# ericzzj1989/BALF

Hardware: NVIDIA B200
Metric: images/sec detect+NMS+top-k @640x480 (higher is better)
Workload: dtype fp16/tf32 operands (11-bit significand), fp32 accumulate

## Files before the change

### balf_b200/csrc/detector_tc.cuh

```cuda
#pragma once
#include <cuda_fp16.h>
#include "detector.cuh"
#include "umma.cuh"

namespace balf {
using namespace umma;

constexpr int kMerge32Ctas = 3;
constexpr int kRc16MinC = 32;
constexpr int TM = 128;
constexpr int NT2 = 256;
constexpr int kMaxSlot = 4;
constexpr int kMaxGemm = 6;

struct TcGemm {
    uint32_t goff;
    uint16_t nblk;
    uint16_t rows;
    uint16_t kb;
    uint16_t bias;
    uint16_t h16;
};
__host__ __device__ constexpr uint32_t tc_eb(int h16) { return h16 == 1 ? 2u : 4u; }
struct TcPlan {
// ... 107 lines not shown
    static constexpr int nslot = PX ? (C == 256 ? 2 : 3) : (C == 256 ? 3 : 2);
    __host__ __device__ static constexpr int rows(int gi) { return gi == BG_WM ? 64 : C; }
    __host__ __device__ static constexpr int K(int gi) { return gi == BG_CONV0 ? tc_kin(CIN) : gi == BG_WM ? 64 : C; }
    __host__ __device__ static constexpr bool bias(int gi) { return gi != BG_WM; }
    __host__ __device__ static constexpr bool h16(int gi) { return gi != BG_CONV0 || CIN >= 8; }
};
template <int CIN, int C, int PX = 0> struct MergeG {
    static constexpr int count = MG_COUNT;
    static constexpr bool x3 = PX != 0;
    static constexpr bool ebias = C == 128 && PX == 0;
    static constexpr bool resident = PX ? C <= 32 : C <= 128;
    static constexpr int cap = 32768;
    static constexpr int nslot = PX ? (C == 64 ? 3 : 2) : (C == 256 ? 2 : 3);
    __host__ __device__ static constexpr int rows(int) { return C; }
    __host__ __device__ static constexpr int K(int gi) { return gi == MG_CONV0 ? tc_kin(CIN) : C; }
    __host__ __device__ static constexpr bool bias(int gi) { return !ebias && gi != MG_PD2A; }
    __host__ __device__ static constexpr bool h16(int gi) {
        return gi == MG_PD2A || gi == MG_PD2B || (gi == MG_CONV0 && CIN >= 8) || ((gi == MG_RC1 || gi == MG_RC2) && (PX || C > kRc16MinC));
    }
};
template <int C, int PX = 0> struct HeadG {
    static constexpr int count = HG_COUNT;
    static constexpr bool x3 = PX != 0;
    static constexpr bool resident = false;
    static constexpr int cap = 32768;
    static constexpr int nslot = 2;
    __host__ __device__ static constexpr int rows(int gi) { return gi == HG_DENSE ? kHeadN : C; }
    __host__ __device__ static constexpr int K(int) { return C; }
    __host__ __device__ static constexpr bool bias(int) { return true; }
    __host__ __device__ static constexpr bool h16(int) { return true; }
};
template <typename G> __host__ __device__ constexpr int g_mode(int gi) { return G::h16(gi) ? (G::x3 ? 2 : 1) : 0; }
template <typename G> __host__ __device__ constexpr uint32_t g_bytes(int gi) {
    return (uint32_t)G::rows(gi) * (G::K(gi) * tc_eb(g_mode<G>(gi)) + (G::bias(gi) ? 32u : 0u));
}
template <typename G> __host__ __device__ constexpr uint32_t g_off(int gi) { uint32_t o = 0; for (int i = 0; i < gi; ++i) o += g_bytes<G>(i); return o; }

constexpr uint32_t kDescHi = (128u >> 4) | (1u << 14);
__device__ __forceinline__ uint64_t desc_of(uint32_t addr, uint32_t lbo) {
    return ((uint64_t)kDescHi << 32) | (uint64_t)(((lbo >> 4) << 16) | ((addr >> 4) & 0x3FFFu));
}

__host__ __device__ constexpr uint32_t make_idesc_f16(int M, int N) { return (1u << 4) | ((uint32_t)(N >> 3) << 17) | ((uint32_t)(M >> 4) << 24); }
__device__ __forceinline__ void mma_f16(uint32_t d_tmem, uint64_t a_desc, uint64_t b_desc, uint32_t idesc, bool accumulate) {
    asm volatile(
        "{\n\t.reg .pred p;\n\tsetp.ne.b32 p, %4, 0;\n\t"
        "tcgen05.mma.cta_group::1.kind::f16 [%0], %1, %2, %3, p;\n\t}"
        :: "r"(d_tmem), "l"(a_desc), "l"(b_desc), "r"(idesc), "r"((uint32_t)accumulate) : "memory");
}
constexpr uint32_t kDescHiSw = (1024u >> 4) | (1u << 14) | (2u << 29);
__device__ __forceinline__ uint64_t desc_sw_of(uint32_t addr) {
    return ((uint64_t)kDescHiSw << 32) | (uint64_t)((1u << 16) | ((addr >> 4) & 0x3FFFu));
}
template <typename G, int GI, bool ASW = false>
__device__ __forceinline__ void issue_linear_t(Ring& r, const TcPlan& p, uint32_t a_addr, uint32_t ones_addr, uint32_t d_tmem, bool first) {
    constexpr int ROWS = G::rows(GI), K = G::K(GI);
    constexpr bool BIAS = G::bias(GI), H16 = G::h16(GI);
    constexpr bool X3 = H16 && G::x3;
    static_assert(!(H16 && ASW), "fp16 operands use the chunk-major layout");
    constexpr int KB = tc_kb(ROWS, K, G::cap, (int)tc_eb(g_mode<G>(GI))), NBLK = K / KB;
    constexpr uint32_t idesc = H16 ? make_idesc_f16(128, ROWS) : make_idesc_tf32(128, ROWS);
    constexpr uint32_t a_lbo = TM * 16u, b_lbo = (uint32_t)ROWS * 16u;
    constexpr int KSTEP = H16 ? 16 : 8, EPC = H16 ? 8 : 4;
    const uint64_t a_desc = ASW ? desc_sw_of(a_addr) : desc_of(a_addr, a_lbo);
#pragma unroll
    for (int b = 0; b < NBLK; ++b) {
        uint32_t w_addr, slot = 0;
        if (G::resident) {
            w_addr = r.wsm + g_off<G>(GI) + (uint32_t)b * ROWS * KB * tc_eb(g_mode<G>(GI));
        } else {
            ring_top_up<G::nslot>(r, p);
            slot = r.cslot;
            mbar_wait(&r.full[slot], r.cpar);
            w_addr = r.wsm + slot * p.slot_bytes;
        }
        const uint64_t b_desc = desc_of(w_addr, b_lbo);
        fence_after_sync();
#pragma unroll
        for (int ks = 0; ks < KB / KSTEP; ++ks) {
            const uint32_t kchunk = (uint32_t)(b * KB) / EPC + (uint32_t)ks * 2u;
            const uint32_t a_off = ASW ? (kchunk / 8u) * (TM * 128u) + (kchunk % 8u) * 16u : kchunk * a_lbo;
            if (H16) mma_f16(d_tmem, a_desc + (a_off >> 4), b_desc + (((uint32_t)ks * 2u * b_lbo) >> 4), idesc, !(first && b == 0 && ks == 0));
            else mma_tf32(d_tmem, a_desc + (a_off >> 4), b_desc + (((uint32_t)ks * 2u * b_lbo) >> 4), idesc, !(first && b == 0 && ks == 0));
            if constexpr (X3) {
                mma_f16(d_tmem, a_desc + ((a_off + (uint32_t)(K / 8) * a_lbo) >> 4), b_desc + (((uint32_t)ks * 2u * b_lbo) >> 4), idesc, true);
                mma_f16(d_tmem, a_desc + (a_off >> 4), b_desc + ((((uint32_t)KB / 8u + (uint32_t)ks * 2u) * b_lbo) >> 4), idesc, true);
            }
        }
        if (BIAS && b + 1 == NBLK)
            mma_tf32(d_tmem, desc_of(ones_addr, TM * 16u), b_desc + ((((uint32_t)KB / EPC) * (X3 ? 2u : 1u) * b_lbo) >> 4), make_idesc_tf32(128, ROWS), true);
        if (!G::resident) { commit(&r.empty[slot]); ring_consumed<G::nslot>(r); }
    }
}

constexpr uint32_t kDescHiMn = ((uint32_t)(TM * 16u) >> 4) | (1u << 14);
__device__ __forceinline__ uint64_t desc_mn_of(uint32_t addr) {
    return ((uint64_t)kDescHiMn << 32) | (uint64_t)(((128u >> 4) << 16) | ((addr >> 4) & 0x3FFFu));
}
template <typename G, int GI, int C>
__device__ __forceinline__ void issue_mix_t(Ring& r, const TcPlan& p, uint32_t y_addr, uint32_t d_tmem) {
    uint32_t w_addr, slot = 0;
    if (G::resident) {
        w_addr = r.wsm + g_off<G>(GI);
    } else {
        ring_top_up<G::nslot>(r, p);
        slot = r.cslot;
        mbar_wait(&r.full[slot], r.cpar);
        w_addr = r.wsm + slot * p.slot_bytes;
    }
    fence_after_sync();
    constexpr uint32_t idesc = make_idesc_f16(64, C) | (1u << 16);
    constexpr uint32_t lo_off = (uint32_t)(C / 8) * TM * 16u;
    const uint64_t w_desc = desc_of(w_addr, 1024u);
    const uint64_t y_desc = desc_mn_of(y_addr);
#pragma unroll
    for (uint32_t u = 0; u < 2; ++u) {
#pragma unroll
        for (uint32_t ks = 0; ks < 4; ++ks) {
            const uint32_t yo = (32u * ks + 16u * u) * 16u;
            mma_f16(d_tmem + ((u * 16u) << 16), w_desc + ((ks * 2u * 1024u) >> 4), y_desc + (yo >> 4), idesc, ks > 0);
            if constexpr (G::x3) {
                mma_f16(d_tmem + ((u * 16u) << 16), w_desc + ((ks * 2u * 1024u) >> 4), y_desc + ((lo_off + yo) >> 4), idesc, true);
                mma_f16(d_tmem + ((u * 16u) << 16), w_desc + ((8192u + ks * 2u * 1024u) >> 4), y_desc + (yo >> 4), idesc, true);
            }
        }
    }
    if (!G::resident) { commit(&r.empty[slot]); ring_consumed<G::nslot>(r); }
}

__device__ __forceinline__ float ex2_approx(float x) {
    float y;
    asm("ex2.approx.ftz.f32 %0, %1;" : "=f"(y) : "f"(x));
    return y;
}
// ... 62 lines not shown
template <int CH>
__device__ __forceinline__ void st_row(uint32_t taddr, const float (&v)[CH]) {
    if constexpr (CH == 16) {
        asm volatile(
            "tcgen05.st.sync.aligned.32x32b.x16.b32 [%0], {%1, %2, %3, %4, %5, %6, %7, %8, %9, %10, %11, %12, %13, %14, %15, %16};"
            :: "r"(taddr), "r"(__float_as_uint(v[0])), "r"(__float_as_uint(v[1])), "r"(__float_as_uint(v[2])), "r"(__float_as_uint(v[3])),
               "r"(__float_as_uint(v[4])), "r"(__float_as_uint(v[5])), "r"(__float_as_uint(v[6])), "r"(__float_as_uint(v[7])),
               "r"(__float_as_uint(v[8])), "r"(__float_as_uint(v[9])), "r"(__float_as_uint(v[10])), "r"(__float_as_uint(v[11])),
               "r"(__float_as_uint(v[12])), "r"(__float_as_uint(v[13])), "r"(__float_as_uint(v[14])), "r"(__float_as_uint(v[15]))
            : "memory");
    } else {
#pragma unroll
        for (int c0 = 0; c0 < CH; c0 += 32) tmem_st32(taddr + c0, *reinterpret_cast<const float (*)[32]>(&v[c0]));
    }
    tmem_st_wait();
}

template <int CH>
__device__ __forceinline__ void row_to_a(const float (&v)[CH], float* region, int row, int col0) {
#pragma unroll
    for (int j = 0; j < CH / 4; ++j)
        *reinterpret_cast<float4*>(region + ((size_t)(col0 / 4 + j) * TM + row) * 4) =
            to_tf32(make_float4(v[4 * j], v[4 * j + 1], v[4 * j + 2], v[4 * j + 3]));
}

__device__ __forceinline__ void split_h2(float a, float b, uint32_t& hi, uint32_t& lo) {
    asm("cvt.rn.satfinite.f16x2.f32 %0, %1, %2;" : "=r"(hi) : "f"(b), "f"(a));
    const float2 f = __half22float2(*reinterpret_cast<const __half2*>(&hi));
    asm("cvt.rn.satfinite.f16x2.f32 %0, %1, %2;" : "=r"(lo) : "f"(b - f.y), "f"(a - f.x));
}
template <int CH, int LOC = 0>
__device__ __forceinline__ void row_to_a16(const float (&v)[CH], float* region, int row, int col0) {
#pragma unroll
    for (int j = 0; j < CH / 8; ++j) {
        uint32_t h[4], l[4];
#pragma unroll
        for (int e = 0; e < 4; ++e) {
            if constexpr (LOC > 0) split_h2(v[8 * j + 2 * e], v[8 * j + 2 * e + 1], h[e], l[e]);
            else asm("cvt.rn.satfinite.f16x2.f32 %0, %1, %2;" : "=r"(h[e]) : "f"(v[8 * j + 2 * e + 1]), "f"(v[8 * j + 2 * e]));
        }
        *reinterpret_cast<uint4*>(region + ((size_t)(col0 / 8 + j) * TM + row) * 4) = make_uint4(h[0], h[1], h[2], h[3]);
        if constexpr (LOC > 0) *reinterpret_cast<uint4*>(region + ((size_t)(LOC + col0 / 8 + j) * TM + row) * 4) = make_uint4(l[0], l[1], l[2], l[3]);
    }
}

__host__ __device__ __forceinline__ int sw_off(int row, int chunk) { return (chunk >> 3) * (TM * 32) + row * 32 + (((chunk & 7) ^ (row & 7)) << 2); }
template <int CH, bool ROUND>
__device__ __forceinline__ void row_to_sw(const float (&v)[CH], float* region, int row, int col0) {
#pragma unroll
    for (int j = 0; j < CH / 4; ++j) {
        float4 o = make_float4(v[4 * j], v[4 * j + 1], v[4 * j + 2], v[4 * j + 3]);
        if (ROUND) o = to_tf32(o);
        *reinterpret_cast<float4*>(region + sw_off(row, col0 / 4 + j)) = o;
    }
}
__device__ __forceinline__ void bulk_store(const float* gdst, uint32_t ssrc, uint32_t bytes) {
    asm volatile("cp.async.bulk.global.shared::cta.bulk_group [%0], [%1], %2;" :: "l"(gdst), "r"(ssrc), "r"(bytes) : "memory");
}
__device__ __forceinline__ void bulk_commit() { asm volatile("cp.async.bulk.commit_group;" ::: "memory"); }
__device__ __forceinline__ void bulk_wait_read() { asm volatile("cp.async.bulk.wait_group.read 0;" ::: "memory"); }
__device__ __forceinline__ void bulk_wait_all() { asm volatile("cp.async.bulk.wait_group 0;" ::: "memory"); }

template <int NG, int NTG = NT2>
__device__ __forceinline__ void group_sync(int grp) {
    if constexpr (NG == 1) __syncthreads();
    else asm volatile("bar.sync %0, %1;" :: "r"(grp + 1), "n"(NTG) : "memory");
}

template <int NG = 1, int TPR = 2>
__device__ __forceinline__ void row_stats(float sum, float sq, float2* xch, int row, int half, int C, float& rstd, float& shift, int grp = 0) {
    if constexpr (TPR == 2) {
        xch[half * TM + row] = make_float2(sum, sq);
        group_sync<NG, TM * TPR>(grp);
        const float2 o = xch[(half ^ 1) * TM + row];
        sum += o.x; sq += o.y;
    } else if constexpr (TPR > 2) {
        xch[half * TM + row] = make_float2(sum, sq);
        group_sync<NG, TM * TPR>(grp);
        sum = 0.f; sq = 0.f;
#pragma unroll
        for (int p = 0; p < TPR; ++p) { const float2 o = xch[p * TM + row]; sum += o.x; sq += o.y; }
    }
    const float inv_c = C == 32 ? 1.0f / 32 : C == 64 ? 1.0f / 64 : C == 128 ? 1.0f / 128 : 1.0f / 256;
    const float mean = sum * inv_c;
    const float var = fmaxf(sq * inv_c - mean * mean, 0.f);
    rstd = rsqrtf(var + 1e-5f);
    shift = -mean * rstd;
}

struct TcShared {
    float* region;
    uint32_t wsm;
    float* ones;
    float2* xch;
    float* vec;
    uint2* sched;
    uint64_t* full;
    uint64_t* empty;
    uint64_t* done;
    uint64_t* aux;
    uint32_t* tmem_slot;
    uint64_t* gdone;
};
constexpr int kMaxGroups = 8;
constexpr uint32_t kSchedEntries = 62;
constexpr uint32_t kOnesBytes = 2 * TM * 16, kXchBytes = 2 * 2 * TM * 8, kVecBytes = (2 * 256 + 64) * 4, kSchedBytes = (kSchedEntries + 2) * 8, kTcTail = 256;
// ... 308 lines not shown
#pragma unroll
                for (int q = 0; q < 4; ++q) {
                    if constexpr (H16 == 2) split_h2(e[2 * q], e[2 * q + 1], h[q], l[q]);
                    else asm("cvt.rn.satfinite.f16x2.f32 %0, %1, %2;" : "=r"(h[q]) : "f"(e[2 * q + 1]), "f"(e[2 * q]));
                }
                *reinterpret_cast<uint4*>(dst + ((size_t)((half * N + j) / 2) * TM + row) * 4) = make_uint4(h[0], h[1], h[2], h[3]);
                if constexpr (H16 == 2)
                    *reinterpret_cast<uint4*>(dst + ((size_t)(CIN / 8 + (half * N + j) / 2) * TM + row) * 4) = make_uint4(l[0], l[1], l[2], l[3]);
            } else {
                *reinterpret_cast<float4*>(dst + ((size_t)(half * N + j) * TM + row) * 4) = to_tf32(c0);
                *reinterpret_cast<float4*>(dst + ((size_t)(half * N + j + 1) * TM + row) * 4) = to_tf32(c1);
            }
        }
    }
}


constexpr int kConv0Off = 64;
template <int CIN, int C>
__device__ __forceinline__ void conv0_stage_weights(const DownW& w, float* vec) {
    for (int i = threadIdx.x; i < CIN * C; i += NT2) vec[kConv0Off + i] = __ldg(w.conv0_w + i);
    for (int i = threadIdx.x; i < C; i += NT2) vec[kConv0Off + CIN * C + i] = __ldg(w.conv0_b + i);
}
template <int CIN, int C, int CH>
__device__ __forceinline__ void conv0_row(const float4 x, const float* vec, int col0, float (&v)[CH]) {
    const float xs[4] = {x.x, x.y, x.z, x.w};
    const float* cw = vec + kConv0Off + col0;
#pragma unroll
    for (int i = 0; i < CH; i += 4) {
        const float4 b = *reinterpret_cast<const float4*>(cw + CIN * C + i);
        unsigned long long a01 = pk2(b.x, b.y), a23 = pk2(b.z, b.w);
#pragma unroll
        for (int k = 0; k < CIN; ++k) {
            const float4 wv = *reinterpret_cast<const float4*>(cw + k * C + i);
            const unsigned long long xk = pk2(xs[k], xs[k]);
            a01 = fma2(pk2(wv.x, wv.y), xk, a01);
            a23 = fma2(pk2(wv.z, wv.w), xk, a23);
        }
        upk2(a01, v[i], v[i + 1]);
        upk2(a23, v[i + 2], v[i + 3]);
#pragma unroll
        for (int j = 0; j < 4; ++j) v[i + j] = fmaxf(v[i + j], 0.f);
    }
}

template <int C, int PX> struct BranchCfg {
    static constexpr int TPR = C == 32 ? 1 : C == 256 ? 4 : 2;
    static constexpr int groups = C == 32 ? 5 : C == 64 ? 2 : 1;
    static constexpr int NTG = TM * TPR;
    static constexpr int CH = C / TPR;
    static constexpr uint32_t region = (uint32_t)TM * C * (PX ? 4u : 2u);
    static constexpr bool park_u = C <= 128;
    static constexpr bool h16_out = C <= 128;
    static constexpr int col_u = 0;
    static constexpr int col_y = park_u ? C : 0;
    static constexpr int ncols = groups * tc_cols(col_y + 2 * C) > 512 ? col_y + 2 * C : tc_cols(col_y + 2 * C);
    static constexpr uint32_t xch = TPR == 1 ? 0u : 2u * TPR * TM * 8u;
    static constexpr int SC = TPR == 1 ? 16 : TPR == 4 ? (CH < 32 ? CH : 32) : (CH > 64 ? 64 : CH);
};

template <int CIN, int C, int BR, int PX>
__device__ __forceinline__ void tc_branch_body(const float* __restrict__ xin, const DownW& w, const TcPlan& plan, const UnitGeom& geo,
                                               float* __restrict__ out, float* __restrict__ scratch, unsigned char* smem) {
    using Cfg = BranchCfg<C, PX>;
    using G = BranchG<CIN, C, PX>;
    constexpr int CH = Cfg::CH, NG = Cfg::groups, TPR = Cfg::TPR, NTG = Cfg::NTG, SC = Cfg::SC;
    constexpr bool X3 = PX != 0;
    constexpr int LOC = X3 ? C / 8 : 0;
    constexpr bool XH = !X3 && CIN >= 8;
    constexpr bool CL16 = !Cfg::h16_out && !X3;
    float* const rt = CL16 ? scratch : out;
    constexpr int XM = XH ? 3 : X3 ? 2 : 1;
    static_assert(NG == 1 || G::resident, "tile groups share resident weights (no ring state per group)");
    static_assert(CH % SC == 0 && SC % 16 == 0, "sub-chunking");
    TcShared s = carve(smem, Cfg::region, plan, NG, Cfg::xch);
    const int grp = NG == 1 ? 0 : (int)(threadIdx.x / NTG);
    const int tid = threadIdx.x - grp * NTG, row = tid & (TM - 1), half = tid >> 7;
    const int vblock = (int)blockIdx.x * NG + grp, vgrid = (int)gridDim.x * NG;
    const int ntiles = (geo.total_units + 1) / 2;
    const uint32_t my_tiles = vblock < ntiles ? (ntiles - 1 - vblock) / vgrid + 1 : 0;
    const DownW::Branch& br = w.br[BR];
    if (grp == 0) {
        for (int i = tid; i < C; i += NTG) { s.vec[i] = __ldg(br.gn_w + i); s.vec[256 + i] = __ldg(br.gn_b + i); }
        for (int i = tid; i < 64; i += NTG) s.vec[512 + i] = __ldg(br.gd_b + i) + 1.0f;
        if constexpr (CIN < 8) {
            for (int i = tid; i < CIN * C; i += NTG) s.vec[kConv0Off + i] = __ldg(w.conv0_w + i);
            for (int i = tid; i < C; i += NTG) s.vec[kConv0Off + CIN * C + i] = __ldg(w.conv0_b + i);
        }
    }
    Ring ring;
    const bool w0 = __shfl_sync(0xffffffffu, tid >> 5, 0) == 0;
    tc_prologue<G::nslot>(s, tc_cols(Cfg::ncols * NG), ring, plan, my_tiles, w0 && grp == 0);
    if (NG > 1) {
        if (grp > 0 && w0 && elect_one()) mbar_wait(&s.full[0], 0);
        s.region += (size_t)grp * (Cfg::region / 4);
        s.xch += (size_t)grp * (Cfg::xch / 8);
        if (grp > 0) s.done = &s.gdone[grp];
    }
    const uint32_t tm = *s.tmem_slot + (uint32_t)(grp * Cfg::ncols);
    const uint32_t lane_base = tm + ((uint32_t)(row & ~31) << 16);
    const uint32_t region_addr = smem_u32(s.region), ones_addr = smem_u32(s.ones);
    const int ug = (row & 31) >> 4, tok = (row >> 5) * 16 + (row & 15);
    const int col0 = half * CH;
    const float* const mix_b1p = s.vec + 512 + tok;
    const int ostride = (BR == 0 ? geo.fw : 1) * C;
    const size_t npix = (size_t)geo.h * geo.w;
    uint32_t phase = 0, xb = 0;
    int it = 0;
    InputPf<CIN, TPR> pf;
    auto coords = [&](int tt, bool& vld, int& im, int& px) {
        const int un = 2 * tt + ug;
        vld = un < geo.total_units;
        im = vld ? fast_div(un, geo.upi, geo.inv_upi) : 0;
        px = unit_pixel<BR>(geo, vld ? un - im * geo.upi : 0, tok);
    };
    auto stats_of = [&](const float (&v)[CH], float& sum, float& sq) {
        unsigned long long s2 = pk2(0.f, 0.f), q2 = pk2(0.f, 0.f);
#pragma unroll
        for (int i = 0; i < CH; i += 2) {
            const unsigned long long x = pk2(v[i], v[i + 1]);
            s2 = add2(s2, x); q2 = fma2(x, x, q2);
        }
        float a, b;
        upk2(s2, a, b); sum = a + b;
        upk2(q2, a, b); sq = a + b;
    };
    bool nvld = false; int nim = 0, npx = 0;
// ... 67 lines not shown
            commit(s.done);
        }
        TC_TRACE(plan, it, 8);
        wait_done_ring<G, NG, NTG>(s.done, phase, ring, plan, w0, grp);
        TC_TRACE(plan, it, 9);
        {
            ld_row<CH>(lane_base + Cfg::col_y + col0, v);
            { float d0, d1; gelu_row<CH, false>(v, d0, d1); }
            st_row<CH>(lane_base + Cfg::col_y + col0, v);
            ld_row<CH>(lane_base + Cfg::col_y + C + col0, v);
            float sum = 0.f, sq = 0.f;
            gelu_row<CH, true>(v, sum, sq);
            row_stats<NG, TPR>(sum, sq, s.xch + (xb++ & 1) * TPR * TM, row, half, C, rstd, shift, grp);
            norm_row<CH>(v, rstd, shift);
#pragma unroll
            for (int i = 0; i < CH; i += 4) {
                const float4 gw = *reinterpret_cast<const float4*>(s.vec + col0 + i), gb = *reinterpret_cast<const float4*>(s.vec + 256 + col0 + i);
                upk2(fma2(pk2(v[i], v[i + 1]), pk2(gw.x, gw.y), pk2(gb.x, gb.y)), v[i], v[i + 1]);
                upk2(fma2(pk2(v[i + 2], v[i + 3]), pk2(gw.z, gw.w), pk2(gb.z, gb.w)), v[i + 2], v[i + 3]);
            }
            row_to_a16<CH, LOC>(v, s.region, row, col0);
        }
        TC_TRACE(plan, it, 10);
        sync_for_mma<NG, NTG>(grp);
        if (w0 && elect_one()) { issue_mix_t<G, BG_WM, C>(ring, plan, region_addr, tm + Cfg::col_y + C); commit(s.done); }
        TC_TRACE(plan, it, 11);
        wait_done_ring<G, NG, NTG>(s.done, phase, ring, plan, w0, grp);
        TC_TRACE(plan, it, 12);
        {
#pragma unroll 1
            for (int c = 0; c < CH; c += SC) {
                float y1[SC], y2[SC];
                ld_row<SC>(lane_base + Cfg::col_y + col0 + c, y1);
                ld_row<SC>(lane_base + Cfg::col_y + C + col0 + c, y2);
                const float mix_b1 = *mix_b1p;
                const unsigned long long b2 = pk2(mix_b1, mix_b1);
#pragma unroll
                for (int i = 0; i < SC; i += 2) upk2(mul2(pk2(y1[i], y1[i + 1]), add2(pk2(y2[i], y2[i + 1]), b2)), y2[i], y2[i + 1]);
                row_to_a16<SC, LOC>(y2, s.region, row, col0 + c);
            }
        }
        TC_TRACE(plan, it, 13);
        sync_for_mma<NG, NTG>(grp);
        if (w0 && elect_one()) { issue_linear_t<G, BG_D2>(ring, plan, region_addr, ones_addr, tm + Cfg::col_y, true); commit(s.done); }
        TC_TRACE(plan, it, 14);
        wait_done_ring<G, NG, NTG>(s.done, phase, ring, plan, w0, grp);
        TC_TRACE(plan, it, 15);
        {
            const bool odd = (threadIdx.x & 1) != 0;
            const size_t own_base = Cfg::h16_out ? ((size_t)img * npix + (pix & ~(TM - 1))) * C * (X3 ? 2 : 1)
                                                 : ((size_t)img * npix + pix) * C;
            const size_t oth_base = __shfl_xor_sync(0xffffffffu, (unsigned long long)own_base, 1);
            const size_t base_a = odd ? oth_base : own_base, base_b = odd ? own_base : oth_base;
            if constexpr (CL16 && CH % 64 == 0) {
                float hv[CH / 2];
#pragma unroll
                for (int c = 0; c < CH; c += SC) {
                    float a[SC];
                    ld_row<SC>(lane_base + Cfg::col_y + col0 + c, a);
#pragma unroll
                    for (int j0 = 0; j0 < SC / 4; j0 += 8) {
                        float4 t8[8];
                        pair_load<8>(reinterpret_cast<const float4*>(orow + c) + j0, valid, t8);
#pragma unroll
                        for (int j = 0; j < 8; j += 2) {
                            pair_unswap(t8[j], t8[j + 1]);
#pragma unroll
                            for (int u2 = 0; u2 < 2; ++u2) {
                                const float4 rr = t8[j + u2];
                                const int i = 4 * (j0 + j + u2);
                                uint32_t h0, h1;
                                asm("cvt.rn.satfinite.f16x2.f32 %0, %1, %2;" : "=r"(h0) : "f"(a[i + 1] + rr.y), "f"(a[i] + rr.x));
                                asm("cvt.rn.satfinite.f16x2.f32 %0, %1, %2;" : "=r"(h1) : "f"(a[i + 3] + rr.w), "f"(a[i + 2] + rr.z));
                                hv[(c + i) / 2] = __uint_as_float(h0);
                                hv[(c + i) / 2 + 1] = __uint_as_float(h1);
                            }
                        }
                    }
                }
                oct_store<CH / 8>(out, (((size_t)img * npix + pix) * C + col0) / 2, ostride / 2, hv, valid);
            } else
#pragma unroll 1
            for (int c = 0; c < CH; c += SC) {
                float a[SC], r[SC];
                ld_row<SC>(lane_base + Cfg::col_y + col0 + c, a);
                if (Cfg::park_u) ld_row<SC>(lane_base + Cfg::col_u + col0 + c, r);
                if constexpr (Cfg::h16_out) {
                    __half* tile = reinterpret_cast<__half*>(out) + own_base + (size_t)(pix & (TM - 1)) * 8;
#pragma unroll
                    for (int j = 0; j < SC / 8; ++j) {
                        uint32_t h[4], l[4];
#pragma unroll
                        for (int e = 0; e < 4; ++e) {
                            float lo, hi;
                            upk2(add2(pk2(a[8 * j + 2 * e], a[8 * j + 2 * e + 1]), pk2(r[8 * j + 2 * e], r[8 * j + 2 * e + 1])), lo, hi);
                            if constexpr (X3) split_h2(lo, hi, h[e], l[e]);
                            else asm("cvt.rn.satfinite.f16x2.f32 %0, %1, %2;" : "=r"(h[e]) : "f"(hi), "f"(lo));
                        }
                        if (valid) {
                            *reinterpret_cast<uint4*>(tile + (size_t)((col0 + c) / 8 + j) * (TM * 8)) = make_uint4(h[0], h[1], h[2], h[3]);
                            if constexpr (X3)
                                *reinterpret_cast<uint4*>(tile + (size_t)(C / 8 + (col0 + c) / 8 + j) * (TM * 8)) = make_uint4(l[0], l[1], l[2], l[3]);
                        }
                    }
                    continue;
                }
                float4 o[SC / 4];
// ... 30 lines not shown
                        *reinterpret_cast<float4*>(out + base_a + 4 * chunk) = to_a;
                        *reinterpret_cast<float4*>(out + base_b + 4 * chunk) = to_b;
                    }
                }
            }
        }
    }
    tc_finish(*s.tmem_slot, tc_cols(Cfg::ncols * NG));
}

template <int CIN, int C, int BR, int PX>
__global__ void __launch_bounds__(BranchCfg<C, PX>::NTG * BranchCfg<C, PX>::groups, 1)
tc_branch_kernel(const float* __restrict__ xin, DownW w, TcPlan plan, UnitGeom geo, float* __restrict__ out, float* __restrict__ scratch) {
    extern __shared__ __align__(1024) unsigned char smem[];
    tc_branch_body<CIN, C, BR, PX>(xin, w, plan, geo, out, scratch, smem);
}


template <int C, int NTH = NT2>
__device__ __forceinline__ void unit_channel_sums(const float* reg, int t, int total_units, float* __restrict__ partial) {
    constexpr int CQ = C / 4, PAIRS = 2 * CQ, TPP = NTH / PAIRS, RPT = 64 / TPP;
    static_assert(TPP >= 2 && TPP <= 16, "group must fit in a warp");
    const int tid = threadIdx.x, pair = tid / TPP, sub = tid % TPP;
    const int uu = pair / CQ, ch = pair % CQ;
    const float4* src = reinterpret_cast<const float4*>(reg) + (size_t)ch * TM + uu * 64 + sub;
    float4 acc = src[0];
#pragma unroll
    for (int i = 1; i < RPT; ++i) {
        const float4 x = src[i * TPP];
        acc.x += x.x; acc.y += x.y; acc.z += x.z; acc.w += x.w;
    }
#pragma unroll
    for (int o = TPP / 2; o >= 1; o >>= 1) {
        acc.x += __shfl_xor_sync(0xffffffffu, acc.x, o);
        acc.y += __shfl_xor_sync(0xffffffffu, acc.y, o);
        acc.z += __shfl_xor_sync(0xffffffffu, acc.z, o);
        acc.w += __shfl_xor_sync(0xffffffffu, acc.w, o);
    }
    const int un = 2 * t + uu;
    if (sub == 0 && un < total_units) *reinterpret_cast<float4*>(partial + (size_t)un * C + ch * 4) = acc;
}

__device__ __forceinline__ int col0_of(int tid, int ch) { return (tid >> 7) * ch; }
template <int C, int PX = 0> struct MergeCfg {
    static constexpr int TPR = 2;
    static constexpr int NT = TM * TPR;
    static constexpr uint32_t xch = 2u * TPR * TM * 8u;
    static constexpr int CH = C / TPR;
    static constexpr bool bulk_uv = C == 128;
    static constexpr uint32_t uv_bytes = (uint32_t)TM * C * (PX ? 4u : 2u);
    static constexpr bool two = C == 128 && PX == 0;
    static constexpr uint32_t r2_off = two ? (uint32_t)TM * C * 2 : (uint32_t)TM * C * 4;
    static constexpr uint32_t region = two ? (uint32_t)TM * C * 4 : (uint32_t)TM * C * 4 + (bulk_uv ? uv_bytes : 0u);
    static constexpr int col_x0 = 0, col_acc = C;
    static constexpr int ncols = tc_cols(2 * C);
    static constexpr int min_ctas = C <= 32 ? 3 : C <= 64 ? 2 : 1;
};

template <int CIN, int C, int PX = 0>
__global__ void __launch_bounds__(MergeCfg<C, PX>::NT, MergeCfg<C, PX>::min_ctas)
tc_merge_kernel(const float* __restrict__ xin, TcPlan plan, UnitGeom geo, const float* __restrict__ uin,
                const float* __restrict__ vin, float* __restrict__ rout, float* __restrict__ qout, float* __restrict__ partial, int r16) {
    extern __shared__ __align__(1024) unsigned char smem[];
    using Cfg = MergeCfg<C, PX>;
    using G = MergeG<CIN, C, PX>;
    constexpr int CH = Cfg::CH, TPR = Cfg::TPR, NTK = Cfg::NT;
    constexpr int HM = PX ? 2 : 1, LOC = PX ? C / 8 : 0;
    constexpr bool XH = PX == 0 && CIN >= 8;
    constexpr int XM = XH ? 3 : HM;
    const TcShared s = carve(smem, Cfg::region, plan, 1, Cfg::xch);
    const int tid = threadIdx.x, row = tid & (TM - 1), half = tid >> 7;
    const int ntiles = (geo.total_units + 1) / 2;
    const uint32_t my_tiles = blockIdx.x < (unsigned)ntiles ? (ntiles - 1 - blockIdx.x) / gridDim.x + 1 : 0;
    Ring ring;
    const bool w0 = warp0_uniform();
    tc_prologue<G::nslot>(s, Cfg::ncols, ring, plan, my_tiles, w0);
    const uint32_t tm = *s.tmem_slot;
    if constexpr (G::ebias) {
        for (int i = tid; i < 4 * C; i += NTK) {
            const float2 e = __ldg(reinterpret_cast<const float2*>(plan.base + plan.ebias_off + (size_t)i * 4));
            s.vec[i] = e.x + e.y;
        }
    }
    const float* const eb = s.vec + col0_of(tid, CH);
    const uint32_t lane_base = tm + ((uint32_t)(row & ~31) << 16);
    const uint32_t region_addr = smem_u32(s.region), ones_addr = smem_u32(s.ones);
    const uint32_t r2_addr = region_addr + Cfg::r2_off;
    uint64_t* const ld_u = s.aux;
    uint64_t* const ld_v = &s.gdone[1];
    constexpr uint32_t kTileBytes = Cfg::uv_bytes;
    const size_t tile_floats = (size_t)kTileBytes / 4;
    uint32_t ld_phase = 0;
    const int ug = row >> 6, tok = row & 63;
    const int col0 = half * CH;
    const size_t npix = (size_t)geo.h * geo.w;
    uint32_t phase = 0, xb = 0;
    int it = 0;
    InputPf<CIN, TPR> pf;
    InputPf<C> pfu;
    auto coords = [&](int tt, bool& vld, int& im, int& px) {
        const int un = 2 * tt + ug;
        vld = un < geo.total_units;
        im = vld ? fast_div(un, geo.upi, geo.inv_upi) : 0;
        px = (vld ? un - im * geo.upi : 0) * 64 + tok;
    };
    if (InputPf<CIN, TPR>::enabled && (int)blockIdx.x < ntiles) {
        bool vld; int im, px;
        coords(blockIdx.x, vld, im, px);
        fetch_input_row<CIN, true, TPR, XH>(xin, npix, (size_t)im, px, vld, half, pf);
    }
    if (Cfg::bulk_uv && (int)blockIdx.x < ntiles && w0 && elect_one()) {
        mbar_expect_tx(ld_u, kTileBytes);
        bulk_load(r2_addr, uin + (size_t)blockIdx.x * tile_floats, kTileBytes, ld_u);
    }
    for (int t = blockIdx.x; t < ntiles; t += gridDim.x, ++it) {
        TC_TRACE(plan, it, 0);
        bool valid; int img, pix;
        coords(t, valid, img, pix);
        const size_t row_off = ((size_t)img * npix + pix) * C + col0;
        float v[CH];
        if (InputPf<CIN, TPR>::enabled) {
            store_input_row<CIN, true, TPR, XM>(pf, s.region, row, half);
            if (t + (int)gridDim.x < ntiles) {
                bool vld; int im, px;
                coords(t + gridDim.x, vld, im, px);
                fetch_input_row<CIN, true, TPR, XH>(xin, npix, (size_t)im, px, vld, half, pf);
            }
        } else {
            load_input_row<CIN, TPR, XM>(xin, npix, (size_t)img, pix, valid, s.region, row, half, PX ? 0 : CIN);
        }
        if (InputPf<C>::enabled) fetch_input_row<C>(uin, npix, (size_t)img, pix, valid, half, pfu);
        TC_TRACE(plan, it, 1);
        sync_for_mma();
        if constexpr (Cfg::bulk_uv) {
            if (w0 && elect_one()) {
                issue_linear_t<G, MG_CONV0>(ring, plan, region_addr, ones_addr, tm + Cfg::col_x0, true);
                mbar_wait(ld_u, ld_phase & 1);
                fence_after_sync();
                issue_linear_t<G, MG_PD2A>(ring, plan, r2_addr, ones_addr, tm + Cfg::col_acc, true);
                commit(s.done);
            }
            wait_done_ring<G>(s.done, phase, ring, plan, w0);
            if (w0 && elect_one()) {
                mbar_expect_tx(ld_v, kTileBytes);
                bulk_load(region_addr, vin + (size_t)t * tile_floats, kTileBytes, ld_v);
                if (!Cfg::two && t + (int)gridDim.x < ntiles) {
                    mbar_expect_tx(ld_u, kTileBytes);
                    bulk_load(r2_addr, uin + (size_t)(t + gridDim.x) * tile_floats, kTileBytes, ld_u);
                }
            }
            ld_row<CH>(lane_base + Cfg::col_x0 + col0, v);
#pragma unroll
            for (int i = 0; i < CH; ++i) v[i] = fmaxf(G::ebias ? v[i] + eb[i] : v[i], 0.f);
            st_row<CH>(lane_base + Cfg::col_x0 + col0, v);
            if (w0 && elect_one()) {
                mbar_wait(ld_v, ld_phase & 1);
                fence_after_sync();
                issue_linear_t<G, MG_PD2B>(ring, plan, region_addr, ones_addr, tm + Cfg::col_acc, false);
                commit(s.done);
            }
            ++ld_phase;
            wait_done_ring<G>(s.done, phase, ring, plan, w0);
        } else {
        if (w0 && elect_one()) { issue_linear_t<G, MG_CONV0>(ring, plan, region_addr, ones_addr, tm + Cfg::col_x0, true); commit(s.done); }
        TC_TRACE(plan, it, 2);
        wait_done_ring<G>(s.done, phase, ring, plan, w0);
        TC_TRACE(plan, it, 3);
        ld_row<CH>(lane_base + Cfg::col_x0 + col0, v);
#pragma unroll
        for (int i = 0; i < CH; ++i) v[i] = fmaxf(v[i], 0.f);
        st_row<CH>(lane_base + Cfg::col_x0 + col0, v);
        if (InputPf<C>::enabled) {
            store_input_row<C, true, 2, HM>(pfu, s.region, row, half);
            fetch_input_row<C>(vin, npix, (size_t)img, pix, valid, half, pfu);
        } else {
            load_input_row<C, TPR, PX ? HM : 3>(uin, npix, (size_t)img, pix, valid, s.region, row, half, 0);
        }
        TC_TRACE(plan, it, 4);
        sync_for_mma();
        if (w0 && elect_one()) { issue_linear_t<G, MG_PD2A>(ring, plan, region_addr, ones_addr, tm + Cfg::col_acc, true); commit(s.done); }
        TC_TRACE(plan, it, 5);
        wait_done_ring<G>(s.done, phase, ring, plan, w0);
        TC_TRACE(plan, it, 6);
        if (InputPf<C>::enabled) store_input_row<C, true, 2, HM>(pfu, s.region, row, half);
        else load_input_row<C, TPR, PX ? HM : 3>(vin, npix, (size_t)img, pix, valid, s.region, row, half, 0);
        TC_TRACE(plan, it, 7);
        sync_for_mma();
        if (w0 && elect_one()) { issue_linear_t<G, MG_PD2B>(ring, plan, region_addr, ones_addr, tm + Cfg::col_acc, false); commit(s.done); }
        TC_TRACE(plan, it, 8);
        wait_done_ring<G>(s.done, phase, ring, plan, w0);
        }
        TC_TRACE(plan, it, 9);
// ... 115 lines not shown
    constexpr bool XH = PX == 0 && CIN >= 8;
    constexpr int XM = XH ? 3 : HM;
    const TcShared s = carve(smem, Cfg::region, plan, 1, Cfg::xch);
    float* const regU = s.region;
    float* const regV = regU + Cfg::uv_bytes / 4;
    float* const regW = regV + Cfg::uv_bytes / 4;
    float* const regQ = regW + (size_t)TM * C;
    float* const regR = regQ;
    float* const regX = regQ + (size_t)TM * C;
    uint64_t* const ld_bar = s.aux;
    const int tid = threadIdx.x, row = tid & (TM - 1), half = tid >> 7;
    const int ntiles = geo.total_units / 2;
    const uint32_t my_tiles = blockIdx.x < (unsigned)ntiles ? (ntiles - 1 - blockIdx.x) / gridDim.x + 1 : 0;
    if constexpr (Cfg::cc0) conv0_stage_weights<CIN, C>(w, s.vec);
    Ring ring;
    const bool w0 = warp0_uniform();
    tc_prologue<G::nslot>(s, Cfg::ncols, ring, plan, my_tiles, w0);
    const uint32_t tm = *s.tmem_slot;
    const uint32_t lane_base = tm + ((uint32_t)(row & ~31) << 16);
    const uint32_t u_addr = smem_u32(regU), v_addr = smem_u32(regV), w_addr = smem_u32(regW), q_addr = smem_u32(regQ);
    const uint32_t x_addr = smem_u32(regX), ones_addr = smem_u32(s.ones);
    const int col0 = half * CH;
    const size_t npix = (size_t)geo.h * geo.w;
    const size_t tile_floats = (size_t)TM * C;
    uint32_t phase = 0, ld_phase = 0;
    auto coords = [&](int tt, int& im, int& px) {
        const int un = 2 * tt + (row >> 6);
        im = fast_div(un, geo.upi, geo.inv_upi);
        px = (un - im * geo.upi) * 64 + (row & 63);
    };
    auto load_tile = [&](int tt) {
        mbar_expect_tx(ld_bar, 2 * Cfg::uv_bytes);
        bulk_load(u_addr, uin + (size_t)tt * (Cfg::uv_bytes / 4), Cfg::uv_bytes, ld_bar);
        bulk_load(v_addr, vin + (size_t)tt * (Cfg::uv_bytes / 4), Cfg::uv_bytes, ld_bar);
    };
    InputPf<CIN> pfx;
    if ((int)blockIdx.x < ntiles) {
        int im, px;
        coords(blockIdx.x, im, px);
        fetch_input_row<CIN, false, 2, XH>(xin, npix, (size_t)im, px, true, half, pfx);
        if (w0 && elect_one()) load_tile(blockIdx.x);
    }
    for (int t = blockIdx.x; t < ntiles; t += gridDim.x) {
        const int nt = t + (int)gridDim.x;
        float v[CH], x0[CH];
        if constexpr (!Cfg::cc0) {
            store_input_row<CIN, false, 2, XM>(pfx, regX, row, half);
            sync_for_mma();
        }
        if (w0 && elect_one()) {
            if constexpr (!Cfg::cc0) issue_linear_t<G, MG_CONV0>(ring, plan, x_addr, ones_addr, tm + Cfg::col_x0, true);
            mbar_wait(ld_bar, ld_phase & 1);
            fence_after_sync();
            issue_linear_t<G, MG_PD2A>(ring, plan, u_addr, ones_addr, tm + Cfg::col_acc, true);
            issue_linear_t<G, MG_PD2B>(ring, plan, v_addr, ones_addr, tm + Cfg::col_acc, false);
            commit(s.done);
            bulk_wait_read();
        }
        ++ld_phase;
        if constexpr (Cfg::cc0) conv0_row<CIN, C, CH>(pfx.v[0], s.vec, col0, x0);
        if (nt < ntiles) {
            int im, px;
            coords(nt, im, px);
            fetch_input_row<CIN, false, 2, XH>(xin, npix, (size_t)im, px, true, half, pfx);
        }
        wait_done_ring<G>(s.done, phase, ring, plan, w0);
        {
            float rstd, shift;
            ld_row<CH>(lane_base + Cfg::col_acc + col0, v);
            if constexpr (!Cfg::cc0) {
                ld_row<CH>(lane_base + Cfg::col_x0 + col0, x0);
#pragma unroll
                for (int i = 0; i < CH; ++i) x0[i] = fmaxf(x0[i], 0.f);
            }
            unsigned long long s2 = pk2(0.f, 0.f), q2 = pk2(0.f, 0.f);
#pragma unroll
            for (int i = 0; i < CH; i += 2) {
                const unsigned long long xz = pk2(x0[i], x0[i + 1]);
                const unsigned long long x1 = add2(pk2(v[i], v[i + 1]), xz);
                s2 = add2(s2, x1);
                q2 = fma2(x1, x1, q2);
                upk2(x1, v[i], v[i + 1]);
                upk2(add2(x1, xz), x0[i], x0[i + 1]);
            }
            if constexpr (PX == 0) {
                uint32_t bq[CH];
#pragma unroll
                for (int i = 0; i < CH; ++i) bq[i] = __float_as_uint(x0[i]) + 0x80u;
                unsigned char* const qb = reinterpret_cast<unsigned char*>(regQ);
#pragma unroll
                for (int j = 0; j < CH / 8; ++j) {
                    uint4 o;
                    o.x = __byte_perm(bq[8 * j], bq[8 * j + 1], 0x7632); o.y = __byte_perm(bq[8 * j + 2], bq[8 * j + 3], 0x7632);
                    o.z = __byte_perm(bq[8 * j + 4], bq[8 * j + 5], 0x7632); o.w = __byte_perm(bq[8 * j + 6], bq[8 * j + 7], 0x7632);
                    *reinterpret_cast<uint4*>(qb + ((size_t)(col0 / 8 + j) * TM + row) * 16) = o;
                }
#pragma unroll
                for (int j = 0; j < CH / 16; ++j) {
                    uint32_t w4[4];
#pragma unroll
                    for (int e = 0; e < 4; ++e) {
                        const uint32_t lo = __byte_perm(bq[16 * j + 4 * e], bq[16 * j + 4 * e + 1], 0x0051);
                        const uint32_t hi = __byte_perm(bq[16 * j + 4 * e + 2], bq[16 * j + 4 * e + 3], 0x0051);
                        w4[e] = __byte_perm(lo, hi, 0x5410);
                    }
                    *reinterpret_cast<uint4*>(qb + (size_t)TM * C * 2 + ((size_t)(col0 / 16 + j) * TM + row) * 16) = make_uint4(w4[0], w4[1], w4[2], w4[3]);
                }
            } else {
                row_to_sw<CH, false>(x0, regQ, row, col0);
            }
            float sum, sq;
            { float a, b; upk2(s2, a, b); sum = a + b; upk2(q2, a, b); sq = a + b; }
            row_stats(sum, sq, s.xch, row, half, C, rstd, shift);
            norm_row<CH>(v, rstd, shift);
            if constexpr (G::h16(MG_RC1)) row_to_a16<CH, LOC>(v, regW, row, col0); else row_to_sw<CH, true>(v, regW, row, col0);
        }
        sync_for_mma();
        if (w0 && elect_one()) {
            issue_linear_t<G, MG_RC1, !G::h16(MG_RC1)>(ring, plan, w_addr, ones_addr, tm + Cfg::col_acc, true);
            commit(s.done);
            if constexpr (PX == 0) bulk_store(qout + (size_t)t * (tile_floats * 3 / 4), q_addr, Cfg::tile_bytes / 4 * 3);
            else bulk_store(qout + (size_t)t * tile_floats, q_addr, Cfg::tile_bytes);
            bulk_commit();
            if (nt < ntiles) load_tile(nt);
        }
        wait_done_ring<G>(s.done, phase, ring, plan, w0);
        ld_row<CH>(lane_base + Cfg::col_acc + col0, v);
#pragma unroll
        for (int i = 0; i < CH; i += 2) {
            float l0, l1;
            upk2(mul2(pk2(v[i], v[i + 1]), pk2(0.2f, 0.2f)), l0, l1);
            v[i] = fmaxf(v[i], l0); v[i + 1] = fmaxf(v[i + 1], l1);
        }
        if constexpr (G::h16(MG_RC1)) row_to_a16<CH, LOC>(v, regW, row, col0); else row_to_sw<CH, true>(v, regW, row, col0);
        sync_for_mma();
        if (w0 && elect_one()) {
            issue_linear_t<G, MG_RC2, !G::h16(MG_RC2)>(ring, plan, w_addr, ones_addr, tm + Cfg::col_acc, true);
            commit(s.done);
            if constexpr (!PX) bulk_wait_read();
        }
        wait_done_ring<G>(s.done, phase, ring, plan, w0);
        ld_row<CH>(lane_base + Cfg::col_acc + col0, v);
        row_to_sw<CH, false>(v, regW, row, col0);
        if constexpr (!PX) {
            __half* rt = reinterpret_cast<__half*>(regR) + (size_t)row * 8;
#pragma unroll
            for (int j = 0; j < CH / 8; ++j) {
                uint32_t h[4];
#pragma unroll
                for (int e = 0; e < 4; ++e)
                    asm("cvt.rn.satfinite.f16x2.f32 %0, %1, %2;" : "=r"(h[e]) : "f"(v[8 * j + 2 * e + 1]), "f"(v[8 * j + 2 * e]));
                *reinterpret_cast<uint4*>(rt + (size_t)(col0 / 8 + j) * (TM * 8)) = make_uint4(h[0], h[1], h[2], h[3]);
            }
        }
        sync_for_mma();
        if (w0 && elect_one()) {
            if constexpr (PX) bulk_store(rout + (size_t)t * tile_floats, w_addr, Cfg::tile_bytes);
            else bulk_store(rout + (size_t)t * (tile_floats / 2), smem_u32(regR), Cfg::uv_bytes);
            bulk_commit();
        }
        {
            constexpr int CQ = C / 4, TPP = NT2 / (2 * CQ), RPT = 64 / TPP;
            const int pair = tid / TPP, sub = tid % TPP;
            const int uu = pair / CQ, ch = pair % CQ;
            float4 acc = *reinterpret_cast<const float4*>(regW + sw_off(uu * 64 + sub, ch));
#pragma unroll
            for (int i = 1; i < RPT; ++i) {
                const float4 x = *reinterpret_cast<const float4*>(regW + sw_off(uu * 64 + sub + i * TPP, ch));
                acc.x += x.x; acc.y += x.y; acc.z += x.z; acc.w += x.w;
            }
#pragma unroll
            for (int o = TPP / 2; o >= 1; o >>= 1) {
                acc.x += __shfl_xor_sync(0xffffffffu, acc.x, o);
                acc.y += __shfl_xor_sync(0xffffffffu, acc.y, o);
                acc.z += __shfl_xor_sync(0xffffffffu, acc.z, o);
                acc.w += __shfl_xor_sync(0xffffffffu, acc.w, o);
            }
            if (sub == 0) *reinterpret_cast<float4*>(partial + (size_t)(2 * t + uu) * C + ch * 4) = acc;
        }
    }
    if (w0 && elect_one()) bulk_wait_all();
    tc_finish(tm, Cfg::ncols);
}

template <int C, int PX = 0>
__global__ void __launch_bounds__(NT2, 1) tc_head_kernel(const float* __restrict__ r, const float* __restrict__ q,
                                                         const float* __restrict__ scale, TcPlan plan, UnitGeom geo, int cell,
                                                         float* __restrict__ logits, float* __restrict__ prob, int r16) {
    extern __shared__ __align__(1024) unsigned char smem[];
    using G = HeadG<C, PX>;
// ... 487 lines not shown
```

Baseline: 5232.

## Store fp16 branch output in 64-byte swizzled layout for MMA operand

Adds a 64-byte-swizzle shared memory descriptor and layout option to the linear MMA issue routine. The first branch's fp16 u output is now written to global memory already in the SW64 swizzled tile layout, using intra-quad shuffles to form 16-byte panel stores. The consuming merge kernels read it as an SW64 A operand. The aim is to avoid bank conflicts and strided chunk-major access when the tensor cores read the operand, and to coalesce the global writes. The cost is extra shuffles and a cross-kernel layout coupling that depends on correct swizzle math.

```diff
diff --git a/balf_b200/csrc/detector_tc.cuh b/balf_b200/csrc/detector_tc.cuh
--- a/balf_b200/csrc/detector_tc.cuh
+++ b/balf_b200/csrc/detector_tc.cuh
@@ -183,17 +183,27 @@
 __device__ __forceinline__ uint64_t desc_sw_of(uint32_t addr) {
     return ((uint64_t)kDescHiSw << 32) | (uint64_t)((1u << 16) | ((addr >> 4) & 0x3FFFu));
 }
-template <typename G, int GI, bool ASW = false>
+constexpr uint32_t kDescHiSw64 = (512u >> 4) | (1u << 14) | (4u << 29);
+__device__ __forceinline__ uint64_t desc_sw64_of(uint32_t addr) {
+    return ((uint64_t)kDescHiSw64 << 32) | (uint64_t)((1u << 16) | ((addr >> 4) & 0x3FFFu));
+}
+enum ALayout {
+    AL_CM = 0,
+    AL_SW128 = 1,
+    AL_SW64 = 2,
+};
+template <typename G, int GI, int AL = AL_CM>
 __device__ __forceinline__ void issue_linear_t(Ring& r, const TcPlan& p, uint32_t a_addr, uint32_t ones_addr, uint32_t d_tmem, bool first) {
     constexpr int ROWS = G::rows(GI), K = G::K(GI);
     constexpr bool BIAS = G::bias(GI), H16 = G::h16(GI);
     constexpr bool X3 = H16 && G::x3;
-    static_assert(!(H16 && ASW), "fp16 operands use the chunk-major layout");
+    static_assert(AL != AL_SW128 || !H16, "the 128-byte panels hold tf32 operands");
+    static_assert(AL != AL_SW64 || (H16 && !X3), "the 64-byte panels hold single-rounded fp16 operands");
     constexpr int KB = tc_kb(ROWS, K, G::cap, (int)tc_eb(g_mode<G>(GI))), NBLK = K / KB;
     constexpr uint32_t idesc = H16 ? make_idesc_f16(128, ROWS) : make_idesc_tf32(128, ROWS);
     constexpr uint32_t a_lbo = TM * 16u, b_lbo = (uint32_t)ROWS * 16u;
     constexpr int KSTEP = H16 ? 16 : 8, EPC = H16 ? 8 : 4;
-    const uint64_t a_desc = ASW ? desc_sw_of(a_addr) : desc_of(a_addr, a_lbo);
+    const uint64_t a_desc = AL == AL_SW128 ? desc_sw_of(a_addr) : AL == AL_SW64 ? desc_sw64_of(a_addr) : desc_of(a_addr, a_lbo);
 #pragma unroll
     for (int b = 0; b < NBLK; ++b) {
         uint32_t w_addr, slot = 0;
@@ -210,7 +220,8 @@
 #pragma unroll
         for (int ks = 0; ks < KB / KSTEP; ++ks) {
             const uint32_t kchunk = (uint32_t)(b * KB) / EPC + (uint32_t)ks * 2u;
-            const uint32_t a_off = ASW ? (kchunk / 8u) * (TM * 128u) + (kchunk % 8u) * 16u : kchunk * a_lbo;
+            const uint32_t a_off = AL == AL_SW128 ? (kchunk / 8u) * (TM * 128u) + (kchunk % 8u) * 16u
+                                 : AL == AL_SW64 ? (kchunk / 4u) * (TM * 64u) + (kchunk % 4u) * 16u : kchunk * a_lbo;
             if (H16) mma_f16(d_tmem, a_desc + (a_off >> 4), b_desc + (((uint32_t)ks * 2u * b_lbo) >> 4), idesc, !(first && b == 0 && ks == 0));
             else mma_tf32(d_tmem, a_desc + (a_off >> 4), b_desc + (((uint32_t)ks * 2u * b_lbo) >> 4), idesc, !(first && b == 0 && ks == 0));
             if constexpr (X3) {
@@ -379,6 +390,31 @@
         float4 o = make_float4(v[4 * j], v[4 * j + 1], v[4 * j + 2], v[4 * j + 3]);
         if (ROUND) o = to_tf32(o);
         *reinterpret_cast<float4*>(region + sw_off(row, col0 / 4 + j)) = o;
+    }
+}
+__host__ __device__ __forceinline__ int sw64_off(int row, int chunk) { return (chunk >> 2) * (TM * 32) + row * 32 + (((chunk & 3) ^ ((row >> 1) & 3)) << 3); }
+template <int C>
+__device__ __forceinline__ void sw64_store(__half* __restrict__ out, int gpix, int chunk0, const uint32_t (&h)[16], bool valid) {
+    const int a = threadIdx.x & 3;
+    uint4 x[4];
+#pragma unroll
+    for (int k = 0; k < 4; ++k) x[k] = make_uint4(h[4 * k], h[4 * k + 1], h[4 * k + 2], h[4 * k + 3]);
+#pragma unroll
+    for (int s = 2; s >= 1; s >>= 1) {
+        const bool up = (a & s) != 0;
+#pragma unroll
+        for (int k = 0; k < 4; ++k) {
+            if ((k & s) != 0) continue;
+            const uint4 snd = up ? x[k] : x[k | s];
+            const uint4 rcv = make_uint4(__shfl_xor_sync(0xffffffffu, snd.x, s), __shfl_xor_sync(0xffffffffu, snd.y, s),
+                                         __shfl_xor_sync(0xffffffffu, snd.z, s), __shfl_xor_sync(0xffffffffu, snd.w, s));
+            if (up) x[k] = rcv; else x[k | s] = rcv;
+        }
+    }
+#pragma unroll
+    for (int i = 0; i < 4; ++i) {
+        const int g = __shfl_sync(0xffffffffu, gpix, (threadIdx.x & 28) | i);
+        if (valid) *reinterpret_cast<uint4*>(out + (size_t)(g & ~(TM - 1)) * C + sw64_off(g & (TM - 1), chunk0 + a)) = x[i];
     }
 }
 __device__ __forceinline__ void bulk_store(const float* gdst, uint32_t ssrc, uint32_t bytes) {
@@ -793,6 +829,7 @@
     static constexpr uint32_t region = (uint32_t)TM * C * (PX ? 4u : 2u);
     static constexpr bool park_u = C <= 128;
     static constexpr bool h16_out = C <= 128;
+    static constexpr bool u_sw64 = h16_out && !PX;
     static constexpr int col_u = 0;
     static constexpr int col_y = park_u ? C : 0;
     static constexpr int ncols = groups * tc_cols(col_y + 2 * C) > 512 ? col_y + 2 * C : tc_cols(col_y + 2 * C);
@@ -810,10 +847,12 @@
     constexpr int LOC = X3 ? C / 8 : 0;
     constexpr bool XH = !X3 && CIN >= 8;
     constexpr bool CL16 = !Cfg::h16_out && !X3;
+    constexpr bool SW64 = BR == 0 && Cfg::u_sw64;
     float* const rt = CL16 ? scratch : out;
     constexpr int XM = XH ? 3 : X3 ? 2 : 1;
     static_assert(NG == 1 || G::resident, "tile groups share resident weights (no ring state per group)");
     static_assert(CH % SC == 0 && SC % 16 == 0, "sub-chunking");
+    static_assert(!SW64 || CH % 32 == 0, "whole 64-byte panels per thread");
     TcShared s = carve(smem, Cfg::region, plan, NG, Cfg::xch);
     const int grp = NG == 1 ? 0 : (int)(threadIdx.x / NTG);
     const int tid = threadIdx.x - grp * NTG, row = tid & (TM - 1), half = tid >> 7;
@@ -987,7 +1026,27 @@
                                                  : ((size_t)img * npix + pix) * C;
             const size_t oth_base = __shfl_xor_sync(0xffffffffu, (unsigned long long)own_base, 1);
             const size_t base_a = odd ? oth_base : own_base, base_b = odd ? own_base : oth_base;
-            if constexpr (CL16 && CH % 64 == 0) {
+            if constexpr (SW64) {
+                constexpr int SP = SC < 32 ? SC : 32;
+                const int gpix = img * (int)npix + pix;
+#pragma unroll 1
+                for (int c = 0; c < CH; c += 32) {
+                    uint32_t h[16];
+#pragma unroll
+                    for (int s = 0; s < 32; s += SP) {
+                        float a[SP], r[SP];
+                        ld_row<SP>(lane_base + Cfg::col_y + col0 + c + s, a);
+                        ld_row<SP>(lane_base + Cfg::col_u + col0 + c + s, r);
+#pragma unroll
+                        for (int e = 0; e < SP / 2; ++e) {
+                            float lo, hi;
+                            upk2(add2(pk2(a[2 * e], a[2 * e + 1]), pk2(r[2 * e], r[2 * e + 1])), lo, hi);
+                            asm("cvt.rn.satfinite.f16x2.f32 %0, %1, %2;" : "=r"(h[s / 2 + e]) : "f"(hi), "f"(lo));
+                        }
+                    }
+                    sw64_store<C>(reinterpret_cast<__half*>(out), gpix, (col0 + c) / 8, h, valid);
+                }
+            } else if constexpr (CL16 && CH % 64 == 0) {
                 float hv[CH / 2];
 #pragma unroll
                 for (int c = 0; c < CH; c += SC) {
@@ -1124,6 +1183,7 @@
     static constexpr bool two = C == 128 && PX == 0;
     static constexpr uint32_t r2_off = two ? (uint32_t)TM * C * 2 : (uint32_t)TM * C * 4;
     static constexpr uint32_t region = two ? (uint32_t)TM * C * 4 : (uint32_t)TM * C * 4 + (bulk_uv ? uv_bytes : 0u);
+    static_assert(r2_off % 512 == 0, "a 64-byte swizzled operand starts on a 512-byte boundary");
     static constexpr int col_x0 = 0, col_acc = C;
     static constexpr int ncols = tc_cols(2 * C);
     static constexpr int min_ctas = C <= 32 ? 3 : C <= 64 ? 2 : 1;
@@ -1209,7 +1269,7 @@
                 issue_linear_t<G, MG_CONV0>(ring, plan, region_addr, ones_addr, tm + Cfg::col_x0, true);
                 mbar_wait(ld_u, ld_phase & 1);
                 fence_after_sync();
-                issue_linear_t<G, MG_PD2A>(ring, plan, r2_addr, ones_addr, tm + Cfg::col_acc, true);
+                issue_linear_t<G, MG_PD2A, BranchCfg<C, PX>::u_sw64 ? AL_SW64 : AL_CM>(ring, plan, r2_addr, ones_addr, tm + Cfg::col_acc, true);
                 commit(s.done);
             }
             wait_done_ring<G>(s.done, phase, ring, plan, w0);
@@ -1431,7 +1491,7 @@
             if constexpr (!Cfg::cc0) issue_linear_t<G, MG_CONV0>(ring, plan, x_addr, ones_addr, tm + Cfg::col_x0, true);
             mbar_wait(ld_bar, ld_phase & 1);
             fence_after_sync();
-            issue_linear_t<G, MG_PD2A>(ring, plan, u_addr, ones_addr, tm + Cfg::col_acc, true);
+            issue_linear_t<G, MG_PD2A, BranchCfg<C, PX>::u_sw64 ? AL_SW64 : AL_CM>(ring, plan, u_addr, ones_addr, tm + Cfg::col_acc, true);
             issue_linear_t<G, MG_PD2B>(ring, plan, v_addr, ones_addr, tm + Cfg::col_acc, false);
             commit(s.done);
             bulk_wait_read();
@@ -1496,7 +1556,7 @@
         }
         sync_for_mma();
         if (w0 && elect_one()) {
-            issue_linear_t<G, MG_RC1, !G::h16(MG_RC1)>(ring, plan, w_addr, ones_addr, tm + Cfg::col_acc, true);
+            issue_linear_t<G, MG_RC1, G::h16(MG_RC1) ? AL_CM : AL_SW128>(ring, plan, w_addr, ones_addr, tm + Cfg::col_acc, true);
             commit(s.done);
             if constexpr (PX == 0) bulk_store(qout + (size_t)t * (tile_floats * 3 / 4), q_addr, Cfg::tile_bytes / 4 * 3);
             else bulk_store(qout + (size_t)t * tile_floats, q_addr, Cfg::tile_bytes);
@@ -1514,7 +1574,7 @@
         if constexpr (G::h16(MG_RC1)) row_to_a16<CH, LOC>(v, regW, row, col0); else row_to_sw<CH, true>(v, regW, row, col0);
         sync_for_mma();
         if (w0 && elect_one()) {
-            issue_linear_t<G, MG_RC2, !G::h16(MG_RC2)>(ring, plan, w_addr, ones_addr, tm + Cfg::col_acc, true);
+            issue_linear_t<G, MG_RC2, G::h16(MG_RC2) ? AL_CM : AL_SW128>(ring, plan, w_addr, ones_addr, tm + Cfg::col_acc, true);
             commit(s.done);
             if constexpr (!PX) bulk_wait_read();
         }
```

New measurement: 5325 (median of 6 runs). 1.02x the previous value.
